# Tai-Wang/Depth-from-Motion

Measured on NVIDIA B200. Metric: frames/sec, higher is better.
Workload: dtype f32 (bf16x2 split operands, fp32 accumulate)

## Files before the change

depth_from_motion_b200/csrc/conv_tc.cuh:

```cuda
#pragma once
#include <cuda.h>
#include <cuda_bf16.h>

#include <algorithm>
#include <cstdlib>
#include <vector>

#include "common.cuh"
#include "simt_kernels.cuh"

namespace dfm {

inline uint16_t bf16_rn_bits(float f) {
  uint32_t u;
  memcpy(&u, &f, 4);
  if ((u & 0x7F800000u) == 0x7F800000u) return (uint16_t)(u >> 16);
  u += 0x7FFFu + ((u >> 16) & 1u);
  return (uint16_t)(u >> 16);
}
inline float bf16_bits_to_float(uint16_t b) {
  uint32_t u = (uint32_t)b << 16;
  float f;
  memcpy(&f, &u, 4);
  return f;
}

enum { TC_S1 = 0, TC_S2 = 1, TC_T = 2 };
constexpr int TC_BX = 8, TC_BY = 16;
constexpr int TC_LOAD_THREADS = 320;
constexpr int TC_THREADS = 128 + TC_LOAD_THREADS + 32;
constexpr int TC_MAXOPS = 9, TC_MAXBLK = 48;
constexpr int TC_ZERO_TAP = 255;

template <int MODE>
struct TcMode;
template <>
struct TcMode<TC_S1> {
  static constexpr int PXB = 10, PYB = 18, PITCH = 10, ROWS = 186, CG = 32, NSTAGE = 4;
  static constexpr int SLOT_BLOCKS = 1, NSLOT = 16;
  __host__ __device__ static int zo_of(int zi, int dz) { return zi + dz; }
  __host__ __device__ static int zi_first(int zo) { return zo - 1; }
  __host__ __device__ static int zi_last(int zo) { return zo + 1; }
  __host__ __device__ static int ptype(int) { return 0; }
};
template <>
struct TcMode<TC_S2> {
  static constexpr int PXB = 17, PYB = 33, PITCH = 9, ROWS = 620, CG = 16, NSTAGE = 3;
  static constexpr int SLOT_BLOCKS = 1, NSLOT = 16;
  __host__ __device__ static int zo_of(int zi, int dz) { return (zi >> 1) + dz; }
  __host__ __device__ static int zi_first(int zo) { return 2 * zo - 1; }
  __host__ __device__ static int zi_last(int zo) { return 2 * zo + 1; }
  __host__ __device__ static int ptype(int zi) { return zi & 1; }
};
template <>
struct TcMode<TC_T> {
  static constexpr int PXB = 9, PYB = 17, PITCH = 9, ROWS = 154, CG = 32, NSTAGE = 4;
  static constexpr int SLOT_BLOCKS = 4, NSLOT = 8;
  __host__ __device__ static int zo_of(int zi, int dz) { return 2 * zi + dz; }
  __host__ __device__ static int zi_first(int zo) { return zo >> 1; }
  __host__ __device__ static int zi_last(int zo) { return (zo + 1) >> 1; }
  __host__ __device__ static int ptype(int) { return 0; }
};

inline int tc_mode_of(const ConvGeom& g) {
  if (g.transposed) return TC_T;
  if (g.sd == 1 && g.sh == 1 && g.sw == 1 && g.pd == 1 && g.ph == 1 && g.pw == 1) return TC_S1;
  if (g.sd == 2 && g.sh == 2 && g.sw == 2 && g.pd == 1 && g.ph == 1 && g.pw == 1 &&
      g.Di % 2 == 0 && g.Hi % 2 == 0 && g.Wi % 2 == 0)
    return TC_S2;
  return -1;
}
inline bool tc_supported(int Cin, int Cout, int ) {
  if (Cin != 32 && Cin != 64) return false;
  const int ncta = 1024 / Cin;
  return Cout % ncta == 0 && Cout <= 64;
}
inline bool tc_geom_supported(const ConvGeom& g) { return tc_mode_of(g) >= 0; }

struct TcOp {
  uint32_t a_off;
  uint32_t b_off;
  uint32_t b_lbo;
  uint16_t blk0, blk1;
  uint32_t nruns;
  uint32_t runs[3];
};
struct TcBlk {
  int8_t dz;
  uint8_t colblk;
  uint8_t tap;
  uint8_t pad;
};
struct TcProgram {
  int nops;
  uint32_t need;
  TcOp ops[TC_MAXOPS];
  TcBlk blks[TC_MAXBLK];
};

template <int MODE>
inline void tc_build_program(int ptype, int Cin, int ncta, uint32_t* w_cursor, TcProgram* pr) {
  using M = TcMode<MODE>;
  pr->nops = 0;
  pr->need = 0;
  int nb = 0;
  auto add_op = [&](int a_rows, std::vector<TcBlk> blks) {
    TcOp& op = pr->ops[pr->nops++];
    op.a_off = (uint32_t)a_rows * 16;
    op.b_off = *w_cursor;
    op.b_lbo = (uint32_t)blks.size() * ncta * 16;
    op.blk0 = (uint16_t)nb;
    for (TcBlk b : blks) pr->blks[nb++] = b;
    op.blk1 = (uint16_t)nb;
    *w_cursor += (uint32_t)(Cin / 8) * op.b_lbo;
    op.nruns = 0;
    size_t i = 0;
    while (i < blks.size()) {
      size_t e = i + 1;
      auto lin = [&](const TcBlk& b) { return (b.dz + 1) * M::SLOT_BLOCKS + b.colblk; };
      while (e < blks.size() && lin(blks[e]) == lin(blks[i]) + (int)(e - i)) ++e;
      const int nblk = (int)(e - i);
      op.runs[op.nruns++] = (uint32_t)nblk | ((uint32_t)i << 4) | ((uint32_t)lin(blks[i]) << 10);
      for (size_t k = i; k < e; ++k) pr->need |= 1u << (blks[k].dz + 1);
      i = e;
    }
  };
  if (MODE == TC_S1) {
    for (int t = 0; t < 9; ++t) {
// ... 70 lines not shown
    std::vector<uint16_t> img((size_t)nsplit * image_bytes / 2);
    const int kch = cin_img / 8;
    for (int s = 0; s < nsplit; ++s)
      for (int t = 0; t < ntypes; ++t)
        for (int o = 0; o < prog[t].nops; ++o) {
          const TcOp& op = prog[t].ops[o];
          const int nblk = op.blk1 - op.blk0;
          for (int kc = 0; kc < kch; ++kc)
            for (int b = 0; b < nblk; ++b)
              for (int j = 0; j < ncta; ++j)
                for (int e = 0; e < 8; ++e) {
                  const int tap = prog[t].blks[op.blk0 + b].tap;
                  if (tap == TC_ZERO_TAP) continue;
                  const int ci = kc * 8 + e + (ks ? s * 16 : 0), co = ks ? j : s * ncta + j;
                  const float w = packed[((size_t)tap * cin + ci) * cout + co];
                  const uint16_t hi = bf16_rn_bits(w);
                  const uint16_t lo = bf16_rn_bits(w - bf16_bits_to_float(hi));
                  const size_t off = (size_t)s * image_bytes / 2 + op.b_off / 2 +
                                     ((size_t)kc * nblk * ncta + (size_t)b * ncta + j) * 8 + e;
                  img[off] = hi;
                  img[off + hi_bytes / 2] = lo;
                }
        }
    if (cudaMalloc(&dev, img.size() * 2) != cudaSuccess ||
        cudaMemcpy(dev, img.data(), img.size() * 2, cudaMemcpyHostToDevice) != cudaSuccess) {
      if (err) *err = "TcWeights: device upload failed";
      release();
      return false;
    }
    return true;
  }
  bool build(const float* packed, int cin, int cout, int m, std::string* err) {
    static const bool no_ks1 = getenv("DFM_NO_KSLICE") != nullptr;
    static const bool ks1 = getenv("DFM_KSLICE_S1") != nullptr;
    if (m == TC_S1) return build_mode<TC_S1>(packed, cin, cout, err,
                                             cin == 64 && cout == 64 && !no_ks1 && ks1);
    if (m == TC_S2) {
      static const bool no_ks = getenv("DFM_NO_KSLICE") != nullptr;
      return build_mode<TC_S2>(packed, cin, cout, err, cout == 64 && !no_ks);
    }
    return build_mode<TC_T>(packed, cin, cout, err);
  }
};

__device__ __forceinline__ uint32_t smem_u32(const void* p) {
  return static_cast<uint32_t>(__cvta_generic_to_shared(p));
}
__device__ __forceinline__ void mbar_init(uint32_t bar, uint32_t count) {
  asm volatile("mbarrier.init.shared::cta.b64 [%0], %1;" ::"r"(bar), "r"(count));
}
__device__ __forceinline__ void mbar_arrive(uint32_t bar) {
  asm volatile("mbarrier.arrive.shared::cta.b64 _, [%0];" ::"r"(bar) : "memory");
}
__device__ __forceinline__ void mbar_wait(uint32_t bar, uint32_t parity, int* err) {
  for (int it = 0; it < (1 << 26); ++it) {
    uint32_t ok;
    asm volatile(
        "{\n\t.reg .pred q;\n\t"
        "mbarrier.try_wait.parity.shared::cta.b64 q, [%1], %2;\n\t"
        "selp.u32 %0, 1, 0, q;\n\t}\n"
        : "=r"(ok)
        : "r"(bar), "r"(parity)
        : "memory");
    if (ok) return;
  }
  *reinterpret_cast<volatile int*>(err) = 1;
  __threadfence_system();
}
__device__ __forceinline__ void mbar_wait_timed(uint32_t bar, uint32_t parity, int* err,
                                                unsigned long long& acc, bool timed) {
  if (!timed) {
    mbar_wait(bar, parity, err);
    return;
  }
  const long long t0 = clock64();
  mbar_wait(bar, parity, err);
  acc += (unsigned long long)(clock64() - t0);
}
__device__ __forceinline__ bool elect_one() {
  uint32_t pred;
  asm volatile(
      "{\n\t.reg .pred p;\n\telect.sync _|p, 0xffffffff;\n\tselp.u32 %0, 1, 0, p;\n\t}\n"
      : "=r"(pred));
  return pred != 0;
}
__device__ __forceinline__ void desc_add(uint64_t& d, uint32_t inc16) {
  asm("{\n\t.reg .b32 lo, hi;\n\tmov.b64 {lo, hi}, %0;\n\tadd.u32 lo, lo, %1;\n\t"
      "mov.b64 %0, {lo, hi};\n\t}\n"
      : "+l"(d)
      : "r"(inc16));
}
__device__ __forceinline__ uint64_t pack64(uint32_t lo, uint32_t hi) {
  return ((uint64_t)hi << 32) | lo;
}
__device__ __forceinline__ void umma_commit(uint32_t bar) {
  asm volatile(
      "tcgen05.commit.cta_group::1.mbarrier::arrive::one.shared::cluster.b64 [%0];" ::"r"(bar)
      : "memory");
}
__device__ __forceinline__ void umma_bf16(uint32_t tmem, uint64_t ad, uint64_t bd,
                                          uint32_t idesc, uint32_t acc) {
  asm volatile(
      "{\n\t.reg .pred p;\n\tsetp.ne.b32 p, %4, 0;\n\t"
      "tcgen05.mma.cta_group::1.kind::f16 [%0], %1, %2, %3, p;\n\t}\n" ::"r"(tmem),
      "l"(ad), "l"(bd), "r"(idesc), "r"(acc)
      : "memory");
}
__device__ __forceinline__ uint64_t umma_desc(uint32_t addr, uint32_t lbo, uint32_t sbo) {
  return (uint64_t)((addr >> 4) & 0x3FFF) | ((uint64_t)((lbo >> 4) & 0x3FFF) << 16) |
         ((uint64_t)((sbo >> 4) & 0x3FFF) << 32) | ((uint64_t)1 << 46);
}
__device__ __forceinline__ uint32_t idesc_bf16(int n) {
  return (1u << 4) | (1u << 7) | (1u << 10) | ((uint32_t)(n >> 3) << 17) | ((128u >> 4) << 24);
}

template <int NC>
__device__ __forceinline__ void tmem_ld(uint32_t taddr, uint32_t* r);
template <>
__device__ __forceinline__ void tmem_ld<32>(uint32_t taddr, uint32_t* r) {
  asm volatile(
      "tcgen05.ld.sync.aligned.32x32b.x32.b32 "
      "{%0,%1,%2,%3,%4,%5,%6,%7,%8,%9,%10,%11,%12,%13,%14,%15,%16,%17,%18,%19,%20,%21,"
      "%22,%23,%24,%25,%26,%27,%28,%29,%30,%31}, [%32];\n"
      : "=r"(r[0]), "=r"(r[1]), "=r"(r[2]), "=r"(r[3]), "=r"(r[4]), "=r"(r[5]), "=r"(r[6]),
        "=r"(r[7]), "=r"(r[8]), "=r"(r[9]), "=r"(r[10]), "=r"(r[11]), "=r"(r[12]),
        "=r"(r[13]), "=r"(r[14]), "=r"(r[15]), "=r"(r[16]), "=r"(r[17]), "=r"(r[18]),
        "=r"(r[19]), "=r"(r[20]), "=r"(r[21]), "=r"(r[22]), "=r"(r[23]), "=r"(r[24]),
        "=r"(r[25]), "=r"(r[26]), "=r"(r[27]), "=r"(r[28]), "=r"(r[29]), "=r"(r[30]),
        "=r"(r[31])
      : "r"(taddr));
}
template <>
__device__ __forceinline__ void tmem_ld<16>(uint32_t taddr, uint32_t* r) {
  asm volatile(
      "tcgen05.ld.sync.aligned.32x32b.x16.b32 "
      "{%0,%1,%2,%3,%4,%5,%6,%7,%8,%9,%10,%11,%12,%13,%14,%15}, [%16];\n"
      : "=r"(r[0]), "=r"(r[1]), "=r"(r[2]), "=r"(r[3]), "=r"(r[4]), "=r"(r[5]), "=r"(r[6]),
        "=r"(r[7]), "=r"(r[8]), "=r"(r[9]), "=r"(r[10]), "=r"(r[11]), "=r"(r[12]),
        "=r"(r[13]), "=r"(r[14]), "=r"(r[15])
      : "r"(taddr));
}

template <int NC>
__device__ __forceinline__ void tmem_zero(uint32_t taddr) {
#pragma unroll
  for (int c = 0; c < NC; c += 16) {
    asm volatile(
        "tcgen05.st.sync.aligned.32x32b.x16.b32 [%0], "
        "{%1,%1,%1,%1,%1,%1,%1,%1,%1,%1,%1,%1,%1,%1,%1,%1};\n" ::"r"(taddr + c),
        "r"(0u)
        : "memory");
  }
}

__device__ __forceinline__ void split_store(const float v[8], uint8_t* hi_dst, uint8_t* lo_dst) {
  uint32_t h[4], l[4];
#pragma unroll
  for (int i = 0; i < 4; ++i) {
    const __nv_bfloat162 hh = __floats2bfloat162_rn(v[2 * i], v[2 * i + 1]);
    const float2 hf = __bfloat1622float2(hh);
    const __nv_bfloat162 ll = __floats2bfloat162_rn(v[2 * i] - hf.x, v[2 * i + 1] - hf.y);
    h[i] = *reinterpret_cast<const uint32_t*>(&hh);
    l[i] = *reinterpret_cast<const uint32_t*>(&ll);
  }
  *reinterpret_cast<uint4*>(hi_dst) = make_uint4(h[0], h[1], h[2], h[3]);
  *reinterpret_cast<uint4*>(lo_dst) = make_uint4(l[0], l[1], l[2], l[3]);
}

#ifndef DFM_LD_VARIANT
#define DFM_LD_VARIANT 0
#endif
__device__ __forceinline__ float4 ld_act(const float4* p) {
#if DFM_LD_VARIANT == 1
  return __ldcg(p);
#elif DFM_LD_VARIANT == 2
  float4 v;
  asm volatile("ld.global.nc.L1::no_allocate.L2::256B.v4.f32 {%0,%1,%2,%3}, [%4];"
               : "=f"(v.x), "=f"(v.y), "=f"(v.z), "=f"(v.w) : "l"(p));
  return v;
#elif DFM_LD_VARIANT == 3
  return __ldcs(p);
#elif DFM_LD_VARIANT == 4
  float4 v;
  asm volatile("ld.global.nc.L1::no_allocate.v4.f32 {%0,%1,%2,%3}, [%4];"
               : "=f"(v.x), "=f"(v.y), "=f"(v.z), "=f"(v.w) : "l"(p));
  return v;
#else
  return __ldg(p);
#endif
}

template <int NT>
struct SrcLoader8 {
  static constexpr bool kTma = false;
  Src s;
  int C, H, W;
  static constexpr int BATCH = 6 / NT;
  struct Raw {
    float4 a[NT][2];
  };
  __device__ __forceinline__ void issue(int z, int y, int x, int c0, Raw& r) const {
    const long long inpl = ((long long)y * W + x) * C + c0, plane = (long long)H * W * C;
#pragma unroll
    for (int t = 0; t < NT; ++t) {
      const float* px = s.t[t].x + term_plane(s.t[t], z) * plane + inpl;
      r.a[t][0] = ld_act(reinterpret_cast<const float4*>(px));
      r.a[t][1] = ld_act(reinterpret_cast<const float4*>(px) + 1);
    }
  }
  __device__ __forceinline__ void finish(const Raw& r, int c0, float v[8]) const {
#pragma unroll
    for (int i = 0; i < 8; ++i) v[i] = 0.f;
#pragma unroll
    for (int t = 0; t < NT; ++t) {
      {
        float u[8] = {r.a[t][0].x, r.a[t][0].y, r.a[t][0].z, r.a[t][0].w,
                      r.a[t][1].x, r.a[t][1].y, r.a[t][1].z, r.a[t][1].w};
        if (s.t[t].scale) {
          const float4 s0 = __ldg(reinterpret_cast<const float4*>(s.t[t].scale + c0));
// ... 209 lines not shown
struct TcWalk {
  long long cur, end;
  int split;
};
__device__ __forceinline__ TcWalk tc_walk_begin(const TcParams& p) {
  TcWalk w;
  const int per_split = gridDim.x / p.nsplit;
  w.split = blockIdx.x % p.nsplit;
  const int r = blockIdx.x / p.nsplit;
  const long long units_col = p.Do / p.z_unit;
  const long long total = (long long)p.tiles_x * p.tiles_y * units_col;
  w.cur = total * r / per_split;
  w.end = total * (r + 1) / per_split;
  return w;
}
__device__ __forceinline__ bool tc_walk_next(const TcParams& p, TcWalk& w, TcItem& it) {
  if (w.cur >= w.end) return false;
  const long long units_col = p.Do / p.z_unit;
  const int col = (int)(w.cur / units_col);
  const long long u0 = w.cur % units_col;
  const long long u1 = min(units_col, u0 + (w.end - w.cur));
  it.split = w.split;
  it.x0 = (col % p.tiles_x) * TC_BX;
  it.y0 = (col / p.tiles_x) * TC_BY;
  it.z_lo = (int)u0 * p.z_unit;
  it.z_hi = (int)u1 * p.z_unit;
  w.cur += u1 - u0;
  return true;
}

template <int MODE, int CIN, int NCTA, class Loader>
__global__ void __launch_bounds__(TC_THREADS, 1) conv_tc_kernel(const __grid_constant__ TcParams p,
                                                                 const __grid_constant__ Loader ld) {
  using M = TcMode<MODE>;
  constexpr bool TMA = Loader::kTma;
  static_assert(!TMA || MODE == TC_S2, "the TMA loader serves the stride-2 brick only");
  constexpr int CG = M::CG < CIN ? M::CG : CIN;
  constexpr int NCH = CG / 8;
  constexpr int NCG = CIN / CG;
  static_assert(!TMA || NCH == 2, "TMA stride-2 stages hold two 8-channel chunks");
  constexpr uint32_t S2_CLS16 = TMA ? TMA_S2_CLSR : TMA_S2_CLS;
  constexpr uint32_t A_LBO = TMA ? TMA_S2_CLS * 16 : M::ROWS * 16;
  constexpr uint32_t A_SBO = M::PITCH * 16;
  constexpr uint32_t A_HL = TMA ? 4 * TMA_S2_CLSR * 16 : NCH * M::ROWS * 16;
  constexpr uint32_t STAGE_BYTES = 2 * A_HL;
  constexpr uint32_t B_SBO = 128;
  constexpr int SLOT_COLS = M::SLOT_BLOCKS * NCTA;
  constexpr bool KSLICE = CIN == 16;
  constexpr int TC_NSLOT = M::NSLOT * SLOT_COLS > 512 ? 512 / SLOT_COLS : M::NSLOT;
  constexpr uint32_t TMEM_COLS = TC_NSLOT * SLOT_COLS;
  constexpr int NPOS = M::PXB * M::PYB;
  constexpr int LGROUPS = 2;
  constexpr int LG_THREADS = TC_LOAD_THREADS / LGROUPS;
  constexpr int NITEM = (NPOS * NCH + LG_THREADS - 1) / LG_THREADS;

  extern __shared__ __align__(1024) uint8_t smem[];
  uint8_t* w_s = smem;
  uint8_t* a_s = smem + p.w_bytes;
  uint64_t* bars = reinterpret_cast<uint64_t*>(a_s + M::NSTAGE * STAGE_BYTES);
  uint32_t* tmem_slot = reinterpret_cast<uint32_t*>(bars + 2 * M::NSTAGE + 2 * M::NSLOT + 1);

  const long long t_kernel0 = clock64();
  const int tid = threadIdx.x, lane = tid & 31;
  const int warp = __shfl_sync(0xffffffffu, tid >> 5, 0);
  const uint32_t bar0 = smem_u32(bars);
  auto full_a = [&](int s) { return bar0 + 8u * s; };
  auto empty_a = [&](int s) { return bar0 + 8u * (M::NSTAGE + s); };
  auto full_acc = [&](int s) { return bar0 + 8u * (2 * M::NSTAGE + s); };
  auto empty_acc = [&](int s) { return bar0 + 8u * (2 * M::NSTAGE + TC_NSLOT + s); };
  constexpr int MMA_WARP = TC_THREADS / 32 - 1;

  const uint32_t w_bar = bar0 + 8u * (2 * M::NSTAGE + 2 * TC_NSLOT);
  if (tid == 0) {
    for (int s = 0; s < M::NSTAGE; ++s) {
      mbar_init(full_a(s), TMA ? 1 : LG_THREADS / 32);
      mbar_init(empty_a(s), 1);
    }
    for (int s = 0; s < TC_NSLOT; ++s) {
      mbar_init(full_acc(s), 1);
      mbar_init(empty_acc(s), 4);
    }
    mbar_init(w_bar, 1);
    asm volatile("fence.mbarrier_init.release.cluster;" ::: "memory");
    const int split = blockIdx.x % p.nsplit;
    const uint8_t* src = p.wimg + (size_t)split * p.w_bytes;
    asm volatile("mbarrier.arrive.expect_tx.shared::cta.b64 _, [%0], %1;" ::"r"(w_bar),
                 "r"(p.w_bytes)
                 : "memory");
    constexpr uint32_t CHUNK = 32768;
    for (uint32_t off = 0; off < p.w_bytes; off += CHUNK) {
      const uint32_t n = min(CHUNK, p.w_bytes - off);
      asm volatile(
          "cp.async.bulk.shared::cluster.global.mbarrier::complete_tx::bytes [%0], [%1], %2, [%3];"
          ::"r"(smem_u32(w_s + off)), "l"(src + off), "r"(n), "r"(w_bar)
          : "memory");
    }
  }
  if (warp == MMA_WARP) {
    asm volatile("tcgen05.alloc.cta_group::1.sync.aligned.shared::cta.b32 [%0], %1;" ::"r"(
                     smem_u32(tmem_slot)),
                 "r"(TMEM_COLS));
    asm volatile("tcgen05.relinquish_alloc_permit.cta_group::1.sync.aligned;");
  }
  asm volatile("tcgen05.fence::before_thread_sync;" ::: "memory");
  __syncthreads();
  asm volatile("tcgen05.fence::after_thread_sync;" ::: "memory");
  const uint32_t tmem_base = *tmem_slot;
  if (warp < 4) {
    for (uint32_t c = 0; c < TMEM_COLS; c += 64)
      tmem_zero<64>(tmem_base + ((uint32_t)(warp * 32) << 16) + c);
    asm volatile("tcgen05.wait::st.sync.aligned;" ::: "memory");
  }
  asm volatile("tcgen05.fence::before_thread_sync;" ::: "memory");
  __syncthreads();
  asm volatile("tcgen05.fence::after_thread_sync;" ::: "memory");

  if constexpr (TMA) {
    if (warp == 4 && lane == 0) {
      constexpr uint32_t STAGE_TX = 8u * 2u * TMA_S2_CLS * 16u;
      uint32_t stage_ctr = 0;
      TcWalk walk = tc_walk_begin(p);
      TcItem it;
      while (tc_walk_next(p, walk, it)) {
        const int zi0 = max(M::zi_first(it.z_lo), 0);
        const int zi1 = min(M::zi_last(it.z_hi - 1), p.Di - 1);
        const int chunk0 = CIN == 16 ? it.split * 2 : 0;
        for (int zi = zi0; zi <= zi1; ++zi) {
#pragma unroll 1
          for (int cg = 0; cg < NCG; ++cg, ++stage_ctr) {
            const int s = stage_ctr % M::NSTAGE;
            mbar_wait(empty_a(s), ((stage_ctr / M::NSTAGE) & 1) ^ 1, p.err);
            asm volatile("mbarrier.arrive.expect_tx.shared::cta.b64 _, [%0], %1;" ::"r"(full_a(s)),
                         "r"(STAGE_TX)
                         : "memory");
            const uint32_t st_addr = smem_u32(a_s + s * STAGE_BYTES);
#pragma unroll
            for (int hl = 0; hl < 2; ++hl) {
#pragma unroll
              for (int cls = 0; cls < 4; ++cls) {
                const int bxp = cls >> 1, byp = cls & 1;
                const int cls_in = (1 - byp) * 2 + (1 - bxp);
                const int slab = ((zi * 2 + hl) * 4 + cls_in) * ld.nch_total + chunk0 + cg * NCH;
                tma_load_4d(st_addr + hl * A_HL + cls * (TMA_S2_CLSR * 16), &ld.map,
                            it.x0 - 1 + bxp, it.y0 - 1 + byp, slab, full_a(s));
              }
            }
          }
        }
      }
    }
  }
  if (TMA && warp >= 4 && warp < MMA_WARP) {
  } else if (warp >= 4 && warp < MMA_WARP) {
    const int lgrp = (warp - 4) & (LGROUPS - 1);
    const int lt = ((warp - 4) / LGROUPS) * 32 + lane;
    const int chunk = lt % NCH;
    uint32_t stage_ctr = 0;
    const bool timed = p.role_cycles != nullptr && tid == 128;
    unsigned long long t_wait_e = 0;
    const long long t_begin = clock64();
    TcWalk walk = tc_walk_begin(p);
    TcItem it;
    while (tc_walk_next(p, walk, it)) {
      int soff[NITEM], gx[NITEM], gy[NITEM];
      bool inb[NITEM], live[NITEM];
#pragma unroll
      for (int k = 0; k < NITEM; ++k) {
        const int i = lt + k * LG_THREADS;
        live[k] = i < NPOS * NCH;
        const int pos = i / NCH;
        const int bx = pos % M::PXB, by = pos / M::PXB;
        int row;
        if (MODE == TC_S1) {
          gx[k] = it.x0 - 1 + bx;
          gy[k] = it.y0 - 1 + by;
          row = by * M::PITCH + bx;
        } else if (MODE == TC_S2) {
          gx[k] = 2 * it.x0 - 1 + bx;
          gy[k] = 2 * it.y0 - 1 + by;
          row = (((bx & 1) * 2 + (by & 1)) * 17 + (by >> 1)) * M::PITCH + (bx >> 1);
        } else {
          gx[k] = it.x0 + bx;
          gy[k] = it.y0 + by;
          row = by * M::PITCH + bx;
        }
        inb[k] = live[k] && gx[k] >= 0 && gx[k] < p.Wi && gy[k] >= 0 && gy[k] < p.Hi;
        soff[k] = (chunk * M::ROWS + row) * 16;
      }
      const int zi0 = max(M::zi_first(it.z_lo), 0);
      const int zi1 = min(M::zi_last(it.z_hi - 1), p.Di - 1);
      for (int zi = zi0; zi <= zi1; ++zi) {
#pragma unroll 1
        for (int cg = 0; cg < NCG; ++cg, ++stage_ctr) {
          if ((int)(stage_ctr & (LGROUPS - 1)) != lgrp) continue;
          const int s = stage_ctr % M::NSTAGE;
          mbar_wait_timed(empty_a(s), ((stage_ctr / M::NSTAGE) & 1) ^ 1, p.err, t_wait_e, timed);
          uint8_t* st = a_s + s * STAGE_BYTES;
          const int c0 = cg * CG + chunk * 8 + (KSLICE ? it.split * CIN : 0);
          constexpr int LB = Loader::BATCH < NITEM ? Loader::BATCH : NITEM;
          if (!(p.dbg & 1))
#pragma unroll
          for (int k0 = 0; k0 < NITEM; k0 += LB) {
            typename Loader::Raw raw[LB];
#pragma unroll
            for (int b = 0; b < LB; ++b)
              if (k0 + b < NITEM && inb[k0 + b] && !(p.dbg & 16))
                ld.issue(zi, gy[k0 + b], gx[k0 + b], c0, raw[b]);
#pragma unroll
            for (int b = 0; b < LB; ++b) {
              if (k0 + b < NITEM && live[k0 + b]) {
                float v[8];
                if (inb[k0 + b]) {
                  ld.finish(raw[b], c0, v);
                } else {
#pragma unroll
                  for (int i = 0; i < 8; ++i) v[i] = 0.f;
                }
                if (!(p.dbg & 32)) split_store(v, st + soff[k0 + b], st + A_HL + soff[k0 + b]);
                else if (v[0] + v[1] + v[2] + v[3] + v[4] + v[5] + v[6] + v[7] == 1.2345f) st[0] = 1;
              }
            }
          }
          if (!(p.dbg & 8)) asm volatile("fence.proxy.async.shared::cta;" ::: "memory");
          __syncwarp();
          if (lane == 0) mbar_arrive(full_a(s));
        }
      }
    }
    if (timed) {
      unsigned long long* rc = p.role_cycles + (size_t)blockIdx.x * 8;
      rc[3] = (unsigned long long)(clock64() - t_begin);
      rc[4] = t_wait_e;
    }
  } else if (warp == MMA_WARP) {
    {
      const bool timed = p.role_cycles != nullptr;
      const bool issuer = lane == 0;
      unsigned long long t_wait_a = 0, t_wait_acc = 0;
      const long long t_begin = clock64();
      mbar_wait(w_bar, 0u, p.err);
      const uint32_t w_base = smem_u32(w_s), a_base = smem_u32(a_s);
      const uint32_t tmem_u = __shfl_sync(0xffffffffu, tmem_base, 0);
      constexpr uint32_t A_LBO16 = A_LBO >> 4, A_HL16 = A_HL >> 4;
      const uint32_t a_desc_hi = (A_SBO >> 4) | (1u << 14);
      const uint32_t b_desc_hi = (B_SBO >> 4) | (1u << 14);
      const uint32_t w_hi16 = p.w_hi_bytes >> 4;
      uint32_t stage_ctr = 0, plane_ctr = 0;
      TcWalk walk = tc_walk_begin(p);
      TcItem it;
      while (tc_walk_next(p, walk, it)) {
        const int zi0 = max(M::zi_first(it.z_lo), 0);
        const int zi1 = min(M::zi_last(it.z_hi - 1), p.Di - 1);
        const uint32_t plane_base = plane_ctr;
        for (int zi = zi0; zi <= zi1; ++zi) {
          const TcProgram& pr = p.prog[M::ptype(zi)];
          uint32_t vmask = 0, fmask = 0, colbase[3];
#pragma unroll
          for (int dz = -1; dz <= 1; ++dz) {
            const int zo = M::zo_of(zi, dz);
            const uint32_t j = plane_base + (uint32_t)(zo - it.z_lo);
            colbase[dz + 1] = (j % TC_NSLOT) * SLOT_COLS;
            if (zo >= it.z_lo && zo < it.z_hi) {
              vmask |= 1u << (dz + 1);
              if (zi == max(M::zi_first(zo), zi0)) {
                fmask |= 1u << (dz + 1);
                mbar_wait_timed(empty_acc(j % TC_NSLOT), ((j / TC_NSLOT) & 1) ^ 1, p.err,
                                t_wait_acc, timed);
              }
            }
          }
          const bool regular = (vmask & pr.need) == pr.need;
          const uint32_t wrapmask = (colbase[1] != colbase[0] + SLOT_COLS ? 1u : 0u) |
                                    (colbase[2] != colbase[1] + SLOT_COLS ? 2u : 0u);
          asm volatile("tcgen05.fence::after_thread_sync;" ::: "memory");
#pragma unroll 1
          for (int cg = 0; cg < NCG; ++cg, ++stage_ctr) {
            const int s = stage_ctr % M::NSTAGE;
            mbar_wait_timed(full_a(s), (stage_ctr / M::NSTAGE) & 1, p.err, t_wait_a, timed);
            asm volatile("tcgen05.fence::after_thread_sync;" ::: "memory");
            const uint32_t a_lo_stage =
                (((a_base + s * STAGE_BYTES) >> 4) & 0x3FFF) | (A_LBO16 << 16);
            bool done = false;
            if constexpr (MODE == TC_S1) {
              constexpr uint32_t B_LBO16 = 3 * NCTA;
              constexpr uint32_t TAP16 = (CIN / 8) * B_LBO16;
              constexpr int NKS = CG / 16;
              const uint32_t b_lo0 = ((w_base >> 4) & 0x3FFF) + (uint32_t)(cg * NCH) * B_LBO16 +
                                     (B_LBO16 << 16);
              const int pa = (vmask & 1u) ? 0 : (vmask & 2u) ? 1 : 2;
              const int pb = (vmask & 4u) ? 3 : (vmask & 2u) ? 2 : 1;
              int first = pa;
              while (first < pb) {
                int last = first + 1;
                while (last < pb && !((wrapmask >> (last - 1)) & 1u)) ++last;
                const uint32_t cb0 = first == 0 ? colbase[0] : first == 1 ? colbase[1] : colbase[2];
                const uint32_t d0 = tmem_u + cb0;
                const uint32_t idesc = idesc_bf16((last - first) * NCTA);
                uint64_t da[NKS][2], db[NKS][2];
#pragma unroll
                for (int ks = 0; ks < NKS; ++ks) {
                  da[ks][0] = pack64(a_lo_stage + 2 * ks * A_LBO16, a_desc_hi);
                  da[ks][1] = pack64(a_lo_stage + 2 * ks * A_LBO16 + A_HL16, a_desc_hi);
                  const uint32_t bl = b_lo0 + 2 * ks * B_LBO16 + (uint32_t)first * NCTA;
                  db[ks][0] = pack64(bl, b_desc_hi);
                  db[ks][1] = pack64(bl + w_hi16, b_desc_hi);
                }
#pragma unroll 1
                for (int tap = 0; tap < 9; ++tap) {
                  if (elect_one()) {
#pragma unroll
                    for (int ks = 0; ks < NKS; ++ks) {
                      umma_bf16(d0, da[ks][0], db[ks][0], idesc, 1u);
                      umma_bf16(d0, da[ks][1], db[ks][0], idesc, 1u);
                      umma_bf16(d0, da[ks][0], db[ks][1], idesc, 1u);
                    }
                  }
                  const uint32_t ainc = (tap == 2 || tap == 5) ? (uint32_t)(M::PITCH - 2) : 1u;
#pragma unroll
                  for (int ks = 0; ks < NKS; ++ks) {
                    desc_add(da[ks][0], ainc);
                    desc_add(da[ks][1], ainc);
                    desc_add(db[ks][0], TAP16);
                    desc_add(db[ks][1], TAP16);
                  }
                }
                first = last;
              }
              done = true;
            }
            if constexpr (MODE == TC_S2) {
              constexpr uint32_t KCH16 = CIN / 8;
// ... 109 lines not shown
                    umma_bf16(d_tmem, dah, dbh, idesc, (fresh && ks == 0) ? 0u : 1u);
                    umma_bf16(d_tmem, dal, dbh, idesc, 1u);
                    umma_bf16(d_tmem, dah, dbl, idesc, 1u);
                  }
                }
              };
              if (regular && fm == 0) {
                constexpr uint32_t SB = M::SLOT_BLOCKS;
                for (uint32_t r = 0; r < op.nruns; ++r) {
                  const uint32_t rc = op.runs[r];
                  const uint32_t nblk = rc & 15u, bs = (rc >> 4) & 63u, lin0 = (rc >> 10) & 15u;
                  uint32_t a = lin0;
                  const uint32_t end = lin0 + nblk;
                  while (a < end) {
                    const uint32_t pl = a / SB;
                    uint32_t b = end;
                    if (pl == 0u) {
                      if (wrapmask & 1u) b = min(b, SB);
                      else if (wrapmask & 2u) b = min(b, 2u * SB);
                    } else if (pl == 1u) {
                      if (wrapmask & 2u) b = min(b, 2u * SB);
                    }
                    const uint32_t cbase = pl == 0u ? colbase[0] : pl == 1u ? colbase[1] : colbase[2];
                    issue(cbase + (a % SB) * NCTA, bs + (a - lin0), b - a, 0u);
                    a = b;
                  }
                }
              } else {
                int b = op.blk0;
                while (b < op.blk1) {
                  const TcBlk bk = pr.blks[b];
                  const uint32_t bit = 1u << (bk.dz + 1);
                  if (!(vmask & bit)) {
                    ++b;
                    continue;
                  }
                  const uint32_t fresh = fm & bit;
                  const uint32_t col0 = colbase[bk.dz + 1] + bk.colblk * NCTA;
                  int e = b + 1;
                  while (e < op.blk1 && (e - b) * NCTA < 256) {
                    const TcBlk bn = pr.blks[e];
                    const uint32_t bitn = 1u << (bn.dz + 1);
                    if (!(vmask & bitn) || ((fm & bitn) != 0) != (fresh != 0) ||
                        colbase[bn.dz + 1] + bn.colblk * NCTA != col0 + (uint32_t)(e - b) * NCTA)
                      break;
                    ++e;
                  }
                  issue(col0, (uint32_t)(b - op.blk0), (uint32_t)(e - b), fresh);
                  b = e;
                }
              }
            }
            }
            if (elect_one()) umma_commit(empty_a(s));
            __syncwarp();
          }
#pragma unroll
          for (int dz = -1; dz <= 1; ++dz) {
            const int zo = M::zo_of(zi, dz);
            if ((vmask >> (dz + 1)) & 1u) {
              if (zi == min(M::zi_last(zo), zi1)) {
                const uint32_t j = plane_base + (uint32_t)(zo - it.z_lo);
                if (elect_one()) umma_commit(full_acc(j % TC_NSLOT));
              }
            }
          }
        }
        plane_ctr += it.z_hi - it.z_lo;
      }
      if (timed && issuer) {
        unsigned long long* rc = p.role_cycles + (size_t)blockIdx.x * 8;
        rc[0] = (unsigned long long)(clock64() - t_begin);
        rc[7] = (unsigned long long)(t_begin - t_kernel0);
        rc[1] = t_wait_a;
        rc[2] = t_wait_acc;
      }
    }
    __syncwarp();
  } else {
    uint32_t plane_ctr = 0;
    const int m = warp * 32 + lane;
    const bool timed = p.role_cycles != nullptr && tid == 0;
    unsigned long long t_wait_f = 0;
    const long long t_begin = clock64();
    constexpr int EW = NCTA > 32 ? 32 : NCTA;
    constexpr int NSUB = NCTA / EW;
    constexpr int NST = KSLICE ? 1 : NCTA;
    float ssum[NST], ssq[NST];
#pragma unroll
    for (int i = 0; i < NST; ++i) ssum[i] = ssq[i] = 0.f;
    int cur_split = -1;
    auto flush_stats = [&]() {
      if (KSLICE || !p.stats || cur_split < 0) return;
#pragma unroll
      for (int i = 0; i < NST; ++i) {
        double a = ssum[i], b = ssq[i];
#pragma unroll
        for (int o = 16; o; o >>= 1) {
          a += __shfl_xor_sync(0xffffffffu, a, o);
          b += __shfl_xor_sync(0xffffffffu, b, o);
        }
        if (lane == 0) {
          atomicAdd(p.stats + 2 * (cur_split * NCTA + i), a);
          atomicAdd(p.stats + 2 * (cur_split * NCTA + i) + 1, b);
        }
        ssum[i] = ssq[i] = 0.f;
      }
    };
    TcWalk walk = tc_walk_begin(p);
    TcItem it;
    while (tc_walk_next(p, walk, it)) {
      cur_split = it.split;
      const int mx = it.x0 + (m & 7), my = it.y0 + (m >> 3);
      const bool ok = mx < p.Mx && my < p.My;
      for (int zo = it.z_lo; zo < it.z_hi; ++zo, ++plane_ctr) {
        const int slot = plane_ctr % TC_NSLOT;
        mbar_wait_timed(full_acc(slot), (plane_ctr / TC_NSLOT) & 1, p.err, t_wait_f, timed);
        asm volatile("tcgen05.fence::after_thread_sync;" ::: "memory");
        if (p.dbg & 2) {
          asm volatile("tcgen05.fence::before_thread_sync;" ::: "memory");
          __syncwarp();
          if (lane == 0) mbar_arrive(empty_acc(slot));
          continue;
        }
#pragma unroll
        for (int cb = 0; cb < M::SLOT_BLOCKS; ++cb) {
#pragma unroll
        for (int sub = 0; sub < NSUB; ++sub) {
          uint32_t r[EW];
          const uint32_t tcol = tmem_base + ((uint32_t)(warp * 32) << 16) + slot * SLOT_COLS +
                                cb * NCTA + sub * EW;
          tmem_ld<EW>(tcol, r);
          asm volatile("tcgen05.wait::ld.sync.aligned;" ::: "memory");
          tmem_zero<EW>(tcol);
          if (cb == M::SLOT_BLOCKS - 1 && sub == NSUB - 1) {
            asm volatile("tcgen05.wait::st.sync.aligned;" ::: "memory");
            asm volatile("tcgen05.fence::before_thread_sync;" ::: "memory");
            __syncwarp();
            if (lane == 0) mbar_arrive(empty_acc(slot));
          }
          if (ok) {
            int xo = mx, yo = my;
            if (MODE == TC_T) {
              xo = 2 * mx + ((cb == 1 || cb == 2) ? 1 : 0);
              yo = 2 * my + (cb >= 2 ? 1 : 0);
            }
            const int ch0 = (KSLICE ? 0 : it.split * NCTA) + sub * EW;
            if (p.addend) {
              const int cls = zo == 0 ? 0 : (zo == p.Do - 1 ? 2 : 1);
              const float4* ad = reinterpret_cast<const float4*>(
                  p.addend + (((long long)cls * p.Ho + yo) * p.Wo + xo) * p.Cout + ch0);
#pragma unroll
              for (int q = 0; q < EW / 4; ++q) {
                const float4 a4 = __ldg(ad + q);
                r[4 * q] = __float_as_uint(__uint_as_float(r[4 * q]) + a4.x);
                r[4 * q + 1] = __float_as_uint(__uint_as_float(r[4 * q + 1]) + a4.y);
                r[4 * q + 2] = __float_as_uint(__uint_as_float(r[4 * q + 2]) + a4.z);
                r[4 * q + 3] = __float_as_uint(__uint_as_float(r[4 * q + 3]) + a4.w);
              }
            }
            if (p.store1) {
              p.out[((long long)zo * p.Ho + yo) * p.Wo + xo] = __uint_as_float(r[0]);
            } else {
              float4* dst = reinterpret_cast<float4*>(
                  p.out + (KSLICE ? it.split * p.slice_stride : 0) +
                  (((long long)zo * p.Ho + yo) * p.Wo + xo) * p.Cout + ch0);
#pragma unroll
              for (int q = 0; q < EW / 4; ++q)
                dst[q] = make_float4(__uint_as_float(r[4 * q]), __uint_as_float(r[4 * q + 1]),
                                     __uint_as_float(r[4 * q + 2]), __uint_as_float(r[4 * q + 3]));
            }
            if constexpr (!KSLICE) {
              if (p.stats) {
                const float wz = (zo >= p.zw_lo && zo < p.zw_hi) ? p.zw : 1.f;
#pragma unroll
                for (int i = 0; i < EW; ++i) {
                  const float v = __uint_as_float(r[i]);
                  ssum[sub * EW + i] = fmaf(wz, v, ssum[sub * EW + i]);
                  ssq[sub * EW + i] = fmaf(wz * v, v, ssq[sub * EW + i]);
                }
              }
            }
          }
        }
        }
      }
      flush_stats();
    }
    if (timed) {
      unsigned long long* rc = p.role_cycles + (size_t)blockIdx.x * 8;
      rc[5] = (unsigned long long)(clock64() - t_begin);
      rc[6] = t_wait_f;
    }
  }

  asm volatile("tcgen05.fence::before_thread_sync;" ::: "memory");
  __syncthreads();
  if (warp == MMA_WARP)
    asm volatile("tcgen05.dealloc.cta_group::1.sync.aligned.b32 %0, %1;" ::"r"(tmem_base),
                 "r"(TMEM_COLS));
}

struct TcErrFlag {
  int* host = nullptr;
  int* dev = nullptr;
  int* get() {
    if (!host) {
      if (cudaHostAlloc(&host, sizeof(int), cudaHostAllocMapped | cudaHostAllocPortable) !=
          cudaSuccess) {
        host = nullptr;
        cudaGetLastError();
        return nullptr;
      }
      *host = 0;
      cudaHostGetDevicePointer(&dev, host, 0);
    }
    return dev;
  }
};
inline TcErrFlag& tc_err_flag() {
  static TcErrFlag f;
  return f;
}
inline int tc_consume_error() {
  TcErrFlag& f = tc_err_flag();
  if (!f.host) return 0;
  const int h = *reinterpret_cast<volatile int*>(f.host);
  if (h) *reinterpret_cast<volatile int*>(f.host) = 0;
  return h;
}
inline int tc_sm_count() {
  int& cached = per_device<int, 1>();
  if (!cached) cudaDeviceGetAttribute(&cached, cudaDevAttrMultiProcessorCount, cur_device());
  return cached;
}

__global__ void __launch_bounds__(256)
kslice_reduce_kernel(const float* __restrict__ part, int nsl, long long V, long long HW,
                     float* __restrict__ out, double* __restrict__ stats, int zw_lo, int zw_hi,
                     float zw) {
  __shared__ double sh[2][16][64];
  const int q = threadIdx.x & 15, r = threadIdx.x >> 4;
  double s[4] = {0, 0, 0, 0}, ss[4] = {0, 0, 0, 0};
  const long long w0 = (long long)zw_lo * HW, w1 = (long long)zw_hi * HW;
  for (long long v = (long long)blockIdx.x * 16 + r; v < V; v += (long long)gridDim.x * 16) {
    float4 a = __ldg(reinterpret_cast<const float4*>(part + v * 64) + q);
    for (int k = 1; k < nsl; ++k) {
      const float4 b = __ldg(reinterpret_cast<const float4*>(part + ((long long)k * V + v) * 64) + q);
      a.x += b.x; a.y += b.y; a.z += b.z; a.w += b.w;
    }
// ... 41 lines not shown
  int zw_lo = 0, zw_hi = 0;
  float zw = 1.f;
  long long slice_stride = 0;
};
template <int MODE, int CIN, int NCTA, class Loader>
bool tc_launch(const Loader& ld, const TcWeights& w, float* out, double* stats,
               const ConvGeom& g, cudaStream_t st, std::string* err, TcOpts opt = TcOpts()) {
  using M = TcMode<MODE>;
  constexpr int CG = M::CG < CIN ? M::CG : CIN;
  constexpr size_t STAGE_BYTES = Loader::kTma ? (size_t)2 * 4 * TMA_S2_CLSR * 16
                                              : (size_t)2 * (CG / 8) * M::ROWS * 16;
  const size_t smem = w.image_bytes + M::NSTAGE * STAGE_BYTES +
                      (2 * M::NSTAGE + 2 * M::NSLOT) * 8 + 16;
  auto kern = conv_tc_kernel<MODE, CIN, NCTA, Loader>;
  struct AttrTag { size_t v = 0; };
  static AttrTag attr_dev[kMaxDevices];
  size_t& attr_smem = attr_dev[cur_device()].v;
  if (smem > attr_smem) {
    if (smem > 232448 ||
        cudaFuncSetAttribute(kern, cudaFuncAttributeMaxDynamicSharedMemorySize, (int)smem) !=
            cudaSuccess) {
      if (err) *err = "conv_tc: cannot reserve " + std::to_string(smem) + " B of shared memory";
      return false;
    }
    attr_smem = smem;
  }
  const int sms = tc_sm_count();
  TcParams p{};
  p.wimg = w.dev;
  p.out = out;
  p.stats = stats;
  p.store1 = opt.store1;
  p.slice_stride = opt.slice_stride;
  p.addend = opt.addend;
  p.zw_lo = opt.zw_lo;
  p.zw_hi = opt.zw_hi;
  p.zw = opt.zw;
  p.Di = g.Di; p.Hi = g.Hi; p.Wi = g.Wi;
  p.Do = g.Do; p.Ho = g.Ho; p.Wo = g.Wo;
  p.Cout = g.Cout;
  p.Mx = MODE == TC_T ? g.Wi : g.Wo;
  p.My = MODE == TC_T ? g.Hi : g.Ho;
  p.tiles_x = (p.Mx + TC_BX - 1) / TC_BX;
  p.tiles_y = (p.My + TC_BY - 1) / TC_BY;
  p.nsplit = w.nsplit;
  p.w_bytes = w.image_bytes;
  p.w_hi_bytes = w.hi_bytes;
  p.prog[0] = w.prog[0];
  p.prog[1] = w.prog[1];
  p.z_unit = MODE == TC_T ? 2 : 1;
  const long long cols = (long long)p.tiles_x * p.tiles_y;
  const long long units = cols * (g.Do / p.z_unit);
  int per_split = std::max(1, sms / p.nsplit);
  per_split = (int)std::min<long long>(per_split, units);
  const int grid = per_split * p.nsplit;
  p.err = tc_err_flag().get();
  static const bool role_dbg = getenv("DFM_TC_ROLE_CYCLES") != nullptr;
  static const int dbg_flags = getenv("DFM_TC_DEBUG") ? atoi(getenv("DFM_TC_DEBUG")) : 0;
  p.dbg = dbg_flags;
  static unsigned long long* role_buf = nullptr;
  if (role_dbg) {
    if (!role_buf) cudaMalloc(&role_buf, 1024 * 8 * sizeof(unsigned long long));
    cudaMemsetAsync(role_buf, 0, 1024 * 8 * sizeof(unsigned long long), st);
    p.role_cycles = role_buf;
  }
  kern<<<grid, TC_THREADS, smem, st>>>(p, ld);
  if (role_dbg) {
    cudaStreamSynchronize(st);
    std::vector<unsigned long long> h((size_t)grid * 8);
    cudaMemcpy(h.data(), role_buf, h.size() * 8, cudaMemcpyDeviceToHost);
    double a[8] = {0};
    for (int b = 0; b < grid; ++b)
      for (int k = 0; k < 8; ++k) a[k] += (double)h[(size_t)b * 8 + k] / grid;
    fprintf(stderr,
            "[tc mode=%d cin=%d ncta=%d grid=%d cols=%lld Do=%d] mma: total %.0f wait_full_a %.0f "
            "wait_empty_acc %.0f | load: total %.0f wait_empty_a %.0f | epi: total %.0f "
            "wait_full_acc %.0f | prologue %.0f\n",
            MODE, CIN, NCTA, grid, cols, g.Do, a[0], a[1], a[2], a[3], a[4], a[5], a[6], a[7]);
  }
  const cudaError_t e = cudaGetLastError();
  if (e != cudaSuccess) {
    if (err) *err = std::string("conv_tc launch: ") + cudaGetErrorString(e);
    return false;
  }
  return true;
}

template <class Loader>
bool tc_dispatch(const Loader& ld, const TcWeights& w, float* out, double* stats,
                 const ConvGeom& g, cudaStream_t st, std::string* err, TcOpts opt = TcOpts()) {
  const int mode = tc_mode_of(g);
  if (mode != w.mode) {
    if (err) *err = "conv_tc: weight image was built for a different conv mode";
    return false;
  }
  if (w.kslice) {
    if ((mode != TC_S2 && mode != TC_S1) || g.Cout != 64 || opt.addend || opt.store1) {
      if (err) *err = "conv_tc: K-slice weights are for plain convs with 64 outputs";
      return false;
    }
    const long long V = (long long)g.Do * g.Ho * g.Wo;
    float* part = tc_kslice_scratch().get((size_t)w.nsplit * V * 64);
    if (!part) {
      if (err) *err = "conv_tc: cannot allocate the K-slice scratch";
      return false;
    }
    TcOpts o2 = opt;
    o2.slice_stride = V * 64;
    bool launched = false;
    if constexpr (Loader::kTma) {
      if (mode == TC_S2) launched = tc_launch<TC_S2, 16, 64, Loader>(ld, w, part, nullptr, g, st, err, o2);
      else if (err) *err = "conv_tc: the TMA loader serves stride-2 convs only";
    } else {
      launched = mode == TC_S2
                     ? tc_launch<TC_S2, 16, 64, Loader>(ld, w, part, nullptr, g, st, err, o2)
                     : tc_launch<TC_S1, 16, 64, Loader>(ld, w, part, nullptr, g, st, err, o2);
    }
    if (!launched) return false;
    const int blocks = (int)std::min<long long>(148 * 8, (V + 15) / 16);
// ... 71 lines not shown
```

Baseline: 164.8.

## Share transposed-conv activation staging across a CTA cluster via DSMEM multicast

For the transposed tensor-core conv, the CTAs that split output channels now run as a thread-block cluster. Each CTA loads only a slice of the input channel chunks and writes the split bf16 hi/lo operands into every cluster peer's shared memory. Stage barriers become cluster-scoped, and MMA completion is multicast to all peers. This removes redundant global loads and bf16 splitting of the same activations across channel-split CTAs, at the cost of cluster scheduling limits and cross-CTA synchronization. The transposed epilogue is also rewritten to shuffle-transpose TMEM results so it issues float4 stores of four channels per pixel.

```diff
diff --git a/depth_from_motion_b200/csrc/conv_tc.cuh b/depth_from_motion_b200/csrc/conv_tc.cuh
--- a/depth_from_motion_b200/csrc/conv_tc.cuh
+++ b/depth_from_motion_b200/csrc/conv_tc.cuh
@@ -70,10 +70,10 @@
     return TC_S2;
   return -1;
 }
-inline bool tc_supported(int Cin, int Cout, int ) {
+inline bool tc_supported(int Cin, int Cout, int transposed) {
   if (Cin != 32 && Cin != 64) return false;
   const int ncta = 1024 / Cin;
-  return Cout % ncta == 0 && Cout <= 64;
+  return Cout % ncta == 0 && Cout <= 64 && (!transposed || Cout >= 2 * ncta);
 }
 inline bool tc_geom_supported(const ConvGeom& g) { return tc_mode_of(g) >= 0; }
 
@@ -250,30 +250,59 @@
 __device__ __forceinline__ void mbar_arrive(uint32_t bar) {
   asm volatile("mbarrier.arrive.shared::cta.b64 _, [%0];" ::"r"(bar) : "memory");
 }
+template <bool CLUSTER = false>
 __device__ __forceinline__ void mbar_wait(uint32_t bar, uint32_t parity, int* err) {
   for (int it = 0; it < (1 << 26); ++it) {
     uint32_t ok;
-    asm volatile(
-        "{\n\t.reg .pred q;\n\t"
-        "mbarrier.try_wait.parity.shared::cta.b64 q, [%1], %2;\n\t"
-        "selp.u32 %0, 1, 0, q;\n\t}\n"
-        : "=r"(ok)
-        : "r"(bar), "r"(parity)
-        : "memory");
+    if constexpr (CLUSTER)
+      asm volatile(
+          "{\n\t.reg .pred q;\n\t"
+          "mbarrier.try_wait.parity.acquire.cluster.shared::cta.b64 q, [%1], %2;\n\t"
+          "selp.u32 %0, 1, 0, q;\n\t}\n"
+          : "=r"(ok)
+          : "r"(bar), "r"(parity)
+          : "memory");
+    else
+      asm volatile(
+          "{\n\t.reg .pred q;\n\t"
+          "mbarrier.try_wait.parity.shared::cta.b64 q, [%1], %2;\n\t"
+          "selp.u32 %0, 1, 0, q;\n\t}\n"
+          : "=r"(ok)
+          : "r"(bar), "r"(parity)
+          : "memory");
     if (ok) return;
   }
   *reinterpret_cast<volatile int*>(err) = 1;
   __threadfence_system();
 }
+template <bool CLUSTER = false>
 __device__ __forceinline__ void mbar_wait_timed(uint32_t bar, uint32_t parity, int* err,
                                                 unsigned long long& acc, bool timed) {
   if (!timed) {
-    mbar_wait(bar, parity, err);
+    mbar_wait<CLUSTER>(bar, parity, err);
     return;
   }
   const long long t0 = clock64();
-  mbar_wait(bar, parity, err);
+  mbar_wait<CLUSTER>(bar, parity, err);
   acc += (unsigned long long)(clock64() - t0);
+}
+__device__ __forceinline__ uint32_t mapa_u32(uint32_t addr, uint32_t rank) {
+  uint32_t r;
+  asm volatile("mapa.shared::cluster.u32 %0, %1, %2;" : "=r"(r) : "r"(addr), "r"(rank));
+  return r;
+}
+__device__ __forceinline__ void st_cluster_v4(uint32_t addr, uint4 v) {
+  asm volatile("st.shared::cluster.v4.b32 [%0], {%1, %2, %3, %4};" ::"r"(addr), "r"(v.x),
+               "r"(v.y), "r"(v.z), "r"(v.w)
+               : "memory");
+}
+__device__ __forceinline__ void mbar_arrive_cluster(uint32_t bar) {
+  asm volatile("mbarrier.arrive.release.cluster.shared::cluster.b64 _, [%0];" ::"r"(bar)
+               : "memory");
+}
+__device__ __forceinline__ void cluster_sync() {
+  asm volatile("barrier.cluster.arrive.release.aligned;\n\tbarrier.cluster.wait.acquire.aligned;"
+               ::: "memory");
 }
 __device__ __forceinline__ bool elect_one() {
   uint32_t pred;
@@ -294,6 +323,13 @@
 __device__ __forceinline__ void umma_commit(uint32_t bar) {
   asm volatile(
       "tcgen05.commit.cta_group::1.mbarrier::arrive::one.shared::cluster.b64 [%0];" ::"r"(bar)
+      : "memory");
+}
+__device__ __forceinline__ void umma_commit_mc(uint32_t bar, uint16_t cta_mask) {
+  asm volatile(
+      "tcgen05.commit.cta_group::1.mbarrier::arrive::one.shared::cluster.multicast::cluster.b64 "
+      "[%0], %1;" ::"r"(bar),
+      "h"(cta_mask)
       : "memory");
 }
 __device__ __forceinline__ void umma_bf16(uint32_t tmem, uint64_t ad, uint64_t bd,
@@ -351,7 +387,25 @@
   }
 }
 
-__device__ __forceinline__ void split_store(const float v[8], uint8_t* hi_dst, uint8_t* lo_dst) {
+__device__ __forceinline__ void quad_transpose16(uint32_t (&r)[16], int lane) {
+#pragma unroll
+  for (int b = 1; b <= 2; b <<= 1) {
+    const bool upper = (lane & b) != 0;
+#pragma unroll
+    for (int t = 0; t < 2; ++t) {
+      const int lo = b == 1 ? 2 * t : t, hi = lo + b;
+#pragma unroll
+      for (int e = 0; e < 4; ++e) {
+        const uint32_t send = upper ? r[4 * lo + e] : r[4 * hi + e];
+        const uint32_t recv = __shfl_xor_sync(0xffffffffu, send, b);
+        if (upper) r[4 * lo + e] = recv;
+        else r[4 * hi + e] = recv;
+      }
+    }
+  }
+}
+
+__device__ __forceinline__ void split_bf16(const float v[8], uint4& hi, uint4& lo) {
   uint32_t h[4], l[4];
 #pragma unroll
   for (int i = 0; i < 4; ++i) {
@@ -361,8 +415,14 @@
     h[i] = *reinterpret_cast<const uint32_t*>(&hh);
     l[i] = *reinterpret_cast<const uint32_t*>(&ll);
   }
-  *reinterpret_cast<uint4*>(hi_dst) = make_uint4(h[0], h[1], h[2], h[3]);
-  *reinterpret_cast<uint4*>(lo_dst) = make_uint4(l[0], l[1], l[2], l[3]);
+  hi = make_uint4(h[0], h[1], h[2], h[3]);
+  lo = make_uint4(l[0], l[1], l[2], l[3]);
+}
+__device__ __forceinline__ void split_store(const float v[8], uint8_t* hi_dst, uint8_t* lo_dst) {
+  uint4 h, l;
+  split_bf16(v, h, l);
+  *reinterpret_cast<uint4*>(hi_dst) = h;
+  *reinterpret_cast<uint4*>(lo_dst) = l;
 }
 
 #ifndef DFM_LD_VARIANT
@@ -678,7 +738,11 @@
   constexpr int NPOS = M::PXB * M::PYB;
   constexpr int LGROUPS = 2;
   constexpr int LG_THREADS = TC_LOAD_THREADS / LGROUPS;
-  constexpr int NITEM = (NPOS * NCH + LG_THREADS - 1) / LG_THREADS;
+  constexpr bool CLUSTER = MODE == TC_T;
+  const int ncl = CLUSTER ? p.nsplit : 1;
+  const int crank = CLUSTER ? (int)(blockIdx.x % p.nsplit) : 0;
+  constexpr int NCH_CTA = CLUSTER ? (NCH + 1) / 2 : NCH;
+  constexpr int NITEM = (NPOS * NCH_CTA + LG_THREADS - 1) / LG_THREADS;
 
   extern __shared__ __align__(1024) uint8_t smem[];
   uint8_t* w_s = smem;
@@ -699,8 +763,8 @@
   const uint32_t w_bar = bar0 + 8u * (2 * M::NSTAGE + 2 * TC_NSLOT);
   if (tid == 0) {
     for (int s = 0; s < M::NSTAGE; ++s) {
-      mbar_init(full_a(s), TMA ? 1 : LG_THREADS / 32);
-      mbar_init(empty_a(s), 1);
+      mbar_init(full_a(s), TMA ? 1 : ncl * (LG_THREADS / 32));
+      mbar_init(empty_a(s), ncl);
     }
     for (int s = 0; s < TC_NSLOT; ++s) {
       mbar_init(full_acc(s), 1);
@@ -739,6 +803,7 @@
   }
   asm volatile("tcgen05.fence::before_thread_sync;" ::: "memory");
   __syncthreads();
+  if constexpr (CLUSTER) cluster_sync();
   asm volatile("tcgen05.fence::after_thread_sync;" ::: "memory");
 
   if constexpr (TMA) {
@@ -780,7 +845,9 @@
   } else if (warp >= 4 && warp < MMA_WARP) {
     const int lgrp = (warp - 4) & (LGROUPS - 1);
     const int lt = ((warp - 4) / LGROUPS) * 32 + lane;
-    const int chunk = lt % NCH;
+    const int nchl = CLUSTER ? (NCH - crank + ncl - 1) / ncl : NCH;
+    static_assert(LG_THREADS % 4 == 0 && LG_THREADS % NCH == 0, "chunk per loader thread");
+    const int chunk = CLUSTER ? crank + (lt % nchl) * ncl : lt % NCH;
     uint32_t stage_ctr = 0;
     const bool timed = p.role_cycles != nullptr && tid == 128;
     unsigned long long t_wait_e = 0;
@@ -793,8 +860,8 @@
 #pragma unroll
       for (int k = 0; k < NITEM; ++k) {
         const int i = lt + k * LG_THREADS;
-        live[k] = i < NPOS * NCH;
-        const int pos = i / NCH;
+        live[k] = i < NPOS * nchl;
+        const int pos = i / nchl;
         const int bx = pos % M::PXB, by = pos / M::PXB;
         int row;
         if (MODE == TC_S1) {
@@ -820,7 +887,8 @@
         for (int cg = 0; cg < NCG; ++cg, ++stage_ctr) {
           if ((int)(stage_ctr & (LGROUPS - 1)) != lgrp) continue;
           const int s = stage_ctr % M::NSTAGE;
-          mbar_wait_timed(empty_a(s), ((stage_ctr / M::NSTAGE) & 1) ^ 1, p.err, t_wait_e, timed);
+          mbar_wait_timed<CLUSTER>(empty_a(s), ((stage_ctr / M::NSTAGE) & 1) ^ 1, p.err, t_wait_e,
+                                   timed);
           uint8_t* st = a_s + s * STAGE_BYTES;
           const int c0 = cg * CG + chunk * 8 + (KSLICE ? it.split * CIN : 0);
           constexpr int LB = Loader::BATCH < NITEM ? Loader::BATCH : NITEM;
@@ -842,16 +910,44 @@
 #pragma unroll
                   for (int i = 0; i < 8; ++i) v[i] = 0.f;
                 }
-                if (!(p.dbg & 32)) split_store(v, st + soff[k0 + b], st + A_HL + soff[k0 + b]);
-                else if (v[0] + v[1] + v[2] + v[3] + v[4] + v[5] + v[6] + v[7] == 1.2345f) st[0] = 1;
+                if (p.dbg & 32) {
+                  if (v[0] + v[1] + v[2] + v[3] + v[4] + v[5] + v[6] + v[7] == 1.2345f) st[0] = 1;
+                } else if constexpr (CLUSTER) {
+                  uint4 h, l;
+                  split_bf16(v, h, l);
+                  const uint32_t dst = smem_u32(st + soff[k0 + b]);
+#pragma unroll
+                  for (int r = 0; r < 4; ++r)
+                    if (r < ncl) {
+                      const uint32_t d = mapa_u32(dst, (uint32_t)r);
+                      st_cluster_v4(d, h);
+                      st_cluster_v4(d + A_HL, l);
+                    }
+                } else {
+                  split_store(v, st + soff[k0 + b], st + A_HL + soff[k0 + b]);
+                }
               }
             }
           }
-          if (!(p.dbg & 8)) asm volatile("fence.proxy.async.shared::cta;" ::: "memory");
+          if (!(p.dbg & 8)) {
+            if constexpr (CLUSTER) asm volatile("fence.proxy.async.shared::cluster;" ::: "memory");
+            else asm volatile("fence.proxy.async.shared::cta;" ::: "memory");
+          }
           __syncwarp();
-          if (lane == 0) mbar_arrive(full_a(s));
+          if constexpr (CLUSTER) {
+            if (lane < ncl) mbar_arrive_cluster(mapa_u32(full_a(s), (uint32_t)lane));
+          } else {
+            if (lane == 0) mbar_arrive(full_a(s));
+          }
         }
       }
+    }
+    if constexpr (CLUSTER) {
+      if (tid == 128)
+        for (uint32_t s = 0; s < (uint32_t)M::NSTAGE && s < stage_ctr; ++s) {
+          const uint32_t last = s + (stage_ctr - 1 - s) / M::NSTAGE * M::NSTAGE;
+          mbar_wait<true>(empty_a(s), (last / M::NSTAGE) & 1, p.err);
+        }
     }
     if (timed) {
       unsigned long long* rc = p.role_cycles + (size_t)blockIdx.x * 8;
@@ -902,7 +998,8 @@
 #pragma unroll 1
           for (int cg = 0; cg < NCG; ++cg, ++stage_ctr) {
             const int s = stage_ctr % M::NSTAGE;
-            mbar_wait_timed(full_a(s), (stage_ctr / M::NSTAGE) & 1, p.err, t_wait_a, timed);
+            mbar_wait_timed<CLUSTER>(full_a(s), (stage_ctr / M::NSTAGE) & 1, p.err, t_wait_a,
+                                     timed);
             asm volatile("tcgen05.fence::after_thread_sync;" ::: "memory");
             const uint32_t a_lo_stage =
                 (((a_base + s * STAGE_BYTES) >> 4) & 0x3FFF) | (A_LBO16 << 16);
@@ -1118,7 +1215,11 @@
               }
             }
             }
-            if (elect_one()) umma_commit(empty_a(s));
+            if constexpr (CLUSTER) {
+              if (elect_one()) umma_commit_mc(empty_a(s), (uint16_t)((1u << ncl) - 1u));
+            } else {
+              if (elect_one()) umma_commit(empty_a(s));
+            }
             __syncwarp();
           }
 #pragma unroll
@@ -1189,6 +1290,48 @@
           if (lane == 0) mbar_arrive(empty_acc(slot));
           continue;
         }
+        if constexpr (MODE == TC_T) {
+          static_assert(EW == 16 && NSUB == 1 && !KSLICE, "transposed epilogue: 16 channels");
+          uint32_t r[M::SLOT_BLOCKS][EW];
+          const uint32_t tslot = tmem_base + ((uint32_t)(warp * 32) << 16) + slot * SLOT_COLS;
+#pragma unroll
+          for (int cb = 0; cb < M::SLOT_BLOCKS; ++cb) tmem_ld<EW>(tslot + cb * NCTA, r[cb]);
+          asm volatile("tcgen05.wait::ld.sync.aligned;" ::: "memory");
+          tmem_zero<SLOT_COLS>(tslot);
+          if (ok && p.stats) {
+            const float wz = (zo >= p.zw_lo && zo < p.zw_hi) ? p.zw : 1.f;
+#pragma unroll
+            for (int cb = 0; cb < M::SLOT_BLOCKS; ++cb)
+#pragma unroll
+              for (int i = 0; i < EW; ++i) {
+                const float v = __uint_as_float(r[cb][i]);
+                ssum[i] = fmaf(wz, v, ssum[i]);
+                ssq[i] = fmaf(wz * v, v, ssq[i]);
+              }
+          }
+          const int ch0 = it.split * NCTA + 4 * (lane & 3);
+#pragma unroll
+          for (int cb = 0; cb < M::SLOT_BLOCKS; ++cb) {
+            quad_transpose16(r[cb], lane);
+#pragma unroll
+            for (int k = 0; k < 4; ++k) {
+              const int ms = warp * 32 + (lane & ~3) + k;
+              const int sx = it.x0 + (ms & 7), sy = it.y0 + (ms >> 3);
+              if (sx < p.Mx && sy < p.My) {
+                const int xo = 2 * sx + ((cb == 1 || cb == 2) ? 1 : 0);
+                const int yo = 2 * sy + (cb >= 2 ? 1 : 0);
+                *reinterpret_cast<float4*>(p.out + (((long long)zo * p.Ho + yo) * p.Wo + xo) * p.Cout +
+                                           ch0) =
+                    make_float4(__uint_as_float(r[cb][4 * k]), __uint_as_float(r[cb][4 * k + 1]),
+                                __uint_as_float(r[cb][4 * k + 2]), __uint_as_float(r[cb][4 * k + 3]));
+              }
+            }
+          }
+          asm volatile("tcgen05.wait::st.sync.aligned;" ::: "memory");
+          asm volatile("tcgen05.fence::before_thread_sync;" ::: "memory");
+          __syncwarp();
+          if (lane == 0) mbar_arrive(empty_acc(slot));
+        } else {
 #pragma unroll
         for (int cb = 0; cb < M::SLOT_BLOCKS; ++cb) {
 #pragma unroll
@@ -1250,6 +1393,7 @@
           }
         }
         }
+        }
       }
       flush_stats();
     }
@@ -1262,6 +1406,7 @@
 
   asm volatile("tcgen05.fence::before_thread_sync;" ::: "memory");
   __syncthreads();
+  if constexpr (CLUSTER) cluster_sync();
   if (warp == MMA_WARP)
     asm volatile("tcgen05.dealloc.cta_group::1.sync.aligned.b32 %0, %1;" ::"r"(tmem_base),
                  "r"(TMEM_COLS));
@@ -1409,6 +1554,36 @@
   const long long cols = (long long)p.tiles_x * p.tiles_y;
   const long long units = cols * (g.Do / p.z_unit);
   int per_split = std::max(1, sms / p.nsplit);
+  cudaLaunchAttribute cl_attr[1];
+  if (MODE == TC_T) {
+    if (opt.addend || opt.store1 || p.nsplit < 2 || p.nsplit > 4) {
+      if (err) *err = "conv_tc: transposed conv: no addend / single-channel store, 32..64 outputs";
+      return false;
+    }
+    cl_attr[0].id = cudaLaunchAttributeClusterDimension;
+    cl_attr[0].val.clusterDim.x = (unsigned)p.nsplit;
+    cl_attr[0].val.clusterDim.y = 1;
+    cl_attr[0].val.clusterDim.z = 1;
+    static int max_clusters[kMaxDevices][5];
+    int& mc = max_clusters[cur_device()][p.nsplit];
+    if (!mc) {
+      cudaLaunchConfig_t q{};
+      q.gridDim = dim3((unsigned)(per_split * p.nsplit));
+      q.blockDim = dim3(TC_THREADS);
+      q.dynamicSmemBytes = smem;
+      q.attrs = cl_attr;
+      q.numAttrs = 1;
+      if (cudaOccupancyMaxActiveClusters(&mc, kern, &q) != cudaSuccess || mc <= 0) {
+        mc = 0;
+        cudaGetLastError();
+        if (err) *err = "conv_tc: no resident cluster of " + std::to_string(p.nsplit) + " CTAs";
+        return false;
+      }
+      if (getenv("DFM_TC_ROLE_CYCLES"))
+        fprintf(stderr, "[tc mode=%d cluster=%d] max active clusters %d\n", MODE, p.nsplit, mc);
+    }
+    per_split = std::min(per_split, mc);
+  }
   per_split = (int)std::min<long long>(per_split, units);
   const int grid = per_split * p.nsplit;
   p.err = tc_err_flag().get();
@@ -1421,7 +1596,21 @@
     cudaMemsetAsync(role_buf, 0, 1024 * 8 * sizeof(unsigned long long), st);
     p.role_cycles = role_buf;
   }
-  kern<<<grid, TC_THREADS, smem, st>>>(p, ld);
+  if (MODE == TC_T) {
+    cudaLaunchConfig_t cfg{};
+    cfg.gridDim = dim3((unsigned)grid);
+    cfg.blockDim = dim3(TC_THREADS);
+    cfg.dynamicSmemBytes = smem;
+    cfg.stream = st;
+    cfg.attrs = cl_attr;
+    cfg.numAttrs = 1;
+    if (cudaLaunchKernelEx(&cfg, kern, p, ld) != cudaSuccess) {
+      if (err) *err = std::string("conv_tc cluster launch: ") + cudaGetErrorString(cudaGetLastError());
+      return false;
+    }
+  } else {
+    kern<<<grid, TC_THREADS, smem, st>>>(p, ld);
+  }
   if (role_dbg) {
     cudaStreamSynchronize(st);
     std::vector<unsigned long long> h((size_t)grid * 8);
```

Result: faster. 167.2, median of 6 (+1.5%).
